# zhangganlin/GlORIE-SLAM

Hardware: AMD Instinct MI355X
Metric: DSPO BA-update iters/sec + rendered rays/sec, 640x480 Replica keyframe graph (higher is better)
Workload: dtype f16 corr/ConvGRU, f32 Jacobians, f64 solve; render: f32 (decoder matmuls as 3-term f16 splits, f32 accumulate); 1 GPU; G8: 8 keyframes, 36 edges, 60x80 (640x480/8), BA itrs=2, DSPO stages alternating, context part of the GRU gates (one map per source keyframe) re-evaluated for all keyframes every 12 steps; multiview_filter.thresh = 0.25 (reference ships 0.01, configs/mono_point_slam.yaml:75: with untrained weights 0.01 rejects > 80 % of every frame and no depth_scale step would reach stage 2); render: 524k-point c; edges_local=36, edges_total=36, hw=4800, keyframes=8, parallelism=single GPU

## Files before the change

### glorie_slam_amd/_lib.py

```python
import ctypes
import os
import threading

import torch

_PKG_DIR = os.path.dirname(os.path.abspath(__file__))
LIB_PATH = os.path.join(_PKG_DIR, "lib", "libglorie_hip.so")

GLORIE_F16, GLORIE_F32 = 0, 1
_STATUS = {0: "GLORIE_OK", -1: "GLORIE_EINVAL", -2: "GLORIE_EHIP", -3: "GLORIE_ENOMEM",
           -4: "GLORIE_EUNSUPPORTED"}

_c_int, _c_f, _vp, _sz = ctypes.c_int, ctypes.c_float, ctypes.c_void_p, ctypes.c_size_t

SIGNATURES = {
    "glorie_version": (ctypes.c_char_p, []),
    "glorie_last_hip_error": (_c_int, []),
    "glorie_ctx_create": (_c_int, [ctypes.POINTER(_vp), _sz]),
    "glorie_ctx_destroy": (_c_int, [_vp]),
    "glorie_ctx_reserve": (_c_int, [_vp, _sz]),
    "glorie_ctx_generation": (ctypes.c_ulonglong, [_vp]),
    "glorie_corr_index_fwd": (_c_int, [_vp, _vp, _vp] + [_c_int] * 7 + [_vp]),
    "glorie_corr_lookup_pyramid": (_c_int, [_vp, _c_int, _vp, _vp] + [_c_int] * 7 + [_vp]),
    "glorie_corr_otf": (_c_int, [_vp, _vp, _c_int, _vp, _vp, _vp, _vp] + [_c_int] * 4 + [_vp]),
    "glorie_corr_otf_encode": (_c_int, [_vp, _vp, _c_int, _vp, _vp, _vp, _vp] + [_c_int] * 4 + [_vp, _vp, _vp, _c_int, _vp]),
    "glorie_altcorr_fwd": (_c_int, [_vp] * 4 + [_c_int] * 8 + [_vp]),
    "glorie_bias_act": (_c_int, [_vp, _c_int, _vp, _vp, _c_int, ctypes.c_long, _c_int, _c_int, _vp]),
    "glorie_gru_glo_terms": (_c_int, [_vp, _c_int, _vp, _vp, _c_int, _vp, _vp, _c_int, _vp, _c_int, _vp, _c_int, _c_int, _vp]),
    "glorie_gru_gate_zr": (_c_int, [_vp, _c_int, _vp, _c_int, _vp, _c_int, _vp, _c_int, _vp, _c_int, _c_int, _c_int, _vp]),
    "glorie_gru_gate_q": (_c_int, [_vp, _c_int, _vp, _c_int, _vp, _c_int, _vp, _c_int, _vp, _c_int, _vp, _c_int, _c_int, _c_int, _vp]),
    "glorie_segment_mean": (_c_int, [_vp, _c_int, _vp, _c_int, _vp, _c_int, _vp, _c_int, _c_int, _c_int, _vp]),
    "glorie_conv3x3_small": (_c_int, [_vp, _c_int, _vp, _c_int, _vp, _vp, _c_int, _c_int, _c_int, ctypes.c_float, _vp, _vp, _c_int, _c_int, _c_int, _vp]),
    "glorie_gru_glo_from_tiles": (_c_int, [_vp, _vp, _vp, _c_int, _vp, _c_int, _c_int, _vp]),
    "glorie_update_bookkeeping": (_c_int, [_vp, _vp, _vp, ctypes.c_long, _vp, _vp, _vp, _vp, _c_int, _c_int, _c_f, _vp, _c_int,
                                           _vp]),
    "glorie_conv_igemm_heads": (_c_int, [_vp, _c_int, _c_int, _vp, _c_int, _c_int, _vp, _vp, _c_int, _c_int, _vp, _vp,
                                         _c_int, _c_int, _c_int, _c_int, _vp]),
    "glorie_conv_upsample": (_c_int, [_vp, _c_int, _c_int, _vp, _vp, _vp, _vp, _vp, _c_int, _c_int, _c_int, _c_int, _vp]),
    "glorie_conv_stencil": (_c_int, [_vp, _vp, _c_int, _c_int, _c_int, ctypes.c_float, _vp, _vp, _c_int, _c_int, _c_int, _vp]),
    "glorie_conv_igemm": (_c_int, [_vp, _c_int, _c_int, _vp, _c_int, _c_int, _vp, _c_int, _c_int, _c_int, _vp,
                                   _c_int, _c_int, _vp, _c_int, _vp, _c_int, _vp, _c_int, _vp, _c_int, _vp, _c_int, _vp,
                                   _c_int, _c_int, _c_int, _vp]),
    "glorie_flow_conv7": (_c_int, [_vp, _vp, _vp, _vp, _c_int, _c_int, _c_int, _c_int, _vp]),
    "glorie_motion": (_c_int, [_vp, _vp, _vp, _vp, _c_int, _c_int, _c_int, ctypes.c_float, _vp]),
    "glorie_motion_padded": (_c_int, [_vp, _vp, _vp, _vp, _c_int, _c_int, _c_int, ctypes.c_float, _vp]),
    "glorie_flow_pad": (_c_int, [_vp, _vp, _c_int, _c_int, _c_int, _vp]),
    "glorie_flow_conv7_padded": (_c_int, [_vp, _vp, _vp, _vp, _c_int, _c_int, _c_int, _c_int, _vp]),
    "glorie_publish_flag": (_c_int, [_vp, _vp, _vp, _vp]),
    "glorie_dspo_prepare": (_c_int, [_vp] * 4 + [_c_int] * 4 + [ctypes.c_float, _c_int, ctypes.c_float, _vp, _vp, _c_int] + [_vp] * 9),
    "glorie_corr_lookup_pyramid_tiled": (_c_int, [_vp, _c_int, _vp, _vp] + [_c_int] * 5 + [_vp]),
    "glorie_corr_build": (_c_int, [_vp] * 5 + [_c_int] * 5 + [_vp]),
    "glorie_corr_lookup_arena": (_c_int, [_vp, _c_int, _vp, _vp, _vp] + [_c_int] * 5 + [_vp]),
    "glorie_corr_lookup_tiled_cl": (_c_int, [_vp, _c_int, _vp, _vp, _c_int, _vp] + [_c_int] * 5 + [_vp]),
    "glorie_corr_dm_level_halfs": (ctypes.c_long, [_c_int, _c_int, _c_int]),
    "glorie_corr_dm_build": (_c_int, [_vp] * 5 + [_c_int] * 5 + [_vp]),
    "glorie_corr_dm_lookup": (_c_int, [_vp, _vp, _vp, _c_int, _c_int, _c_int, _c_int, _vp, _vp, _vp, _vp, _c_int, _vp]),
    "glorie_valid_depth_mask": (_c_int, [_vp] * 4 + [_c_int] * 4 + [ctypes.c_float, _c_int, _vp, _vp, _vp]),
    "glorie_reproject": (_c_int, [_vp] * 7 + [_c_int] * 3 + [_vp]),
    "glorie_reproject_motion": (_c_int, [_vp] * 9 + [_c_int] * 3 + [ctypes.c_float, _vp]),
    "glorie_frame_distance": (_c_int, [_vp] * 6 + [_c_int] * 3 + [_c_f, _vp]),
    "glorie_iproj": (_c_int, [_vp] * 4 + [_c_int] * 3 + [_vp]),
    "glorie_depth_filter": (_c_int, [_vp] * 6 + [_c_int] * 4 + [_vp]),
    "glorie_cvx_upsample": (_c_int, [_vp] * 4 + [_c_int] * 5 + [_vp]),
    "glorie_cvx_upsample_nhwc": (_c_int, [_vp, _vp, _vp, _c_int, _vp, _c_int, _c_int, _c_int, _c_int, _vp]),
    "glorie_ba": (_c_int, [_vp] * 10 + [_c_int] * 8 + [_c_f, _c_f, _c_int, _c_int, _vp, _vp, _vp]),
    "glorie_ba_build_system": (_c_int, [_vp] * 10 + [_c_int] * 8 + [_vp, _vp]),
    "glorie_ba_solve_update": (_c_int, [_vp] * 5 + [_c_int] * 7 + [_c_f, _c_f, _c_int, _c_int] + [_vp] * 4),
    "glorie_ba_pack_system": (_c_int, [_vp, _vp, _c_int, _c_int, _vp]),
    "glorie_comm_unique_id": (_c_int, [_vp]),
    "glorie_comm_init": (_c_int, [_vp, _vp, _c_int, _c_int]),
    "glorie_comm_destroy": (_c_int, [_vp]),
    "glorie_comm_world": (_c_int, [_vp]),
    "glorie_allreduce_normal_eq": (_c_int, [_vp, _vp, _sz, _vp]),
    "glorie_allgather_rows": (_c_int, [_vp, _vp, _vp, _sz, _vp]),
    "glorie_dspo_scale_shift": (_c_int, [_vp] * 14 + [_c_int] * 6 + [_c_f, _c_f, _c_f, _vp, _vp]),
    "glorie_knn_build": (_c_int, [_vp, _vp, _c_int, _c_f, _c_int, _vp, _vp, _vp, _vp]),
    "glorie_knn_query": (_c_int, [_vp, _vp, _vp, _vp, _c_int, _c_int, _c_f, _vp, _vp, _vp, _vp, _vp]),
    "glorie_idw_gather": (_c_int, [_vp, _vp, _vp, _vp, _c_int, _c_int, _c_int, _c_f, _vp, _c_int,
                                   _c_int, _vp, _vp, _vp, _vp]),
    "glorie_knn_query_image": (_c_int, [_vp, _vp, _vp, _vp, _c_int, _c_int, _c_f, _vp, _vp, _vp, _vp, _c_int, _c_int,
                                        _vp]),
    "glorie_knn_query_weights": (_c_int, [_vp, _vp, _vp, _vp, _c_int, _c_f, _vp, _vp, _vp, _vp, _c_int, _c_int, _c_int, _c_int,
                                          _c_int, _vp, _vp, _vp]),
    "glorie_idw_gather2": (_c_int, [_vp, _vp, _vp, _vp, _vp, _c_int, _c_int, _c_int, _c_f, _vp, _c_int,
                                    _c_int, _vp, _vp, _vp, _vp, _vp]),
    "glorie_decoder_pack_floats": (_sz, []),
    "glorie_render_mlp": (_c_int, [_vp] * 10 + [_c_int, _vp, _vp, _c_int, _vp, _vp]),
    "glorie_composite": (_c_int, [_vp, _vp, _c_int, _c_int, _c_f, _vp, _vp, _vp, _vp, _vp]),
    "glorie_ray_samples": (_c_int, [_vp] * 5 + [_c_int, _c_int, _c_f, _c_f] + [_vp] * 6),
    "glorie_ray_samples_camera": (_c_int, [_vp, _c_int, ctypes.c_long] + [_vp] * 3 + [_c_int, _c_int, _c_f, _c_f] + [_vp] * 6),
    "glorie_proj_depth": (_c_int, [_vp, _vp, ctypes.c_long, _vp, _c_f, _c_f, _c_f, _c_f, _c_int, _c_int, _vp, _vp]),
# ... 162 lines not shown
```

### glorie_slam_amd/csrc/conv.hip

```cpp
#include <hip/hip_runtime.h>
#include <stdint.h>
#include <stdlib.h>
#include <string.h>
#include <type_traits>
#include "common.hiph"

namespace glorie {

typedef __attribute__((ext_vector_type(8))) _Float16 f16x8;
typedef __attribute__((ext_vector_type(4))) _Float16 f16x4;
typedef __attribute__((ext_vector_type(4))) float f32x4;

enum { EPI_BIAS_ACT = 0, EPI_GRU_ZR = 1, EPI_GRU_Q = 2, EPI_GLO = 3, EPI_HEADS = 4, EPI_UPSAMPLE = 5 };
enum { CACT_NONE = 0, CACT_RELU = 1, CACT_SIGMOID = 2 };

struct ConvArgs {
  const _Float16* xa; int xa_stride; int cha;
  const _Float16* xb; int xb_stride; int chb;
  const _Float16* w;
  int taps, npad, nout;
  long P; int H, W, HW;
  _Float16* out; int out_stride;
  _Float16* out2; int out2_stride;
  const float* terms; int terms_stride; int act;
// ... 427 lines not shown
      o = __fadd_rn(o, __fmul_rn(round_prob(e[k] / sum, a.up_f32 != 0), nb[k]));
    outv[j] = o;
  }
  float* dst = a.up_out + (size_t)frame * 64 * a.HW + (size_t)(8 * y + asub) * (8 * a.W) + 8 * x + hb * 4;
  *reinterpret_cast<float4*>(dst) = make_float4(outv[0], outv[1], outv[2], outv[3]);
}

template <int EPI, int NB, int BK, int NW, int ST, int MB = 4>
__global__ __launch_bounds__(64 * NW, (ST == 1 && MB * NB <= 16) ? 3 : 2) void conv_igemm_kernel(ConvArgs a) {
  constexpr int TN = 32 * MB;
  static_assert(ST == 1 || ST == 2, "LDS stages");
#if defined(__HIP_DEVICE_COMPILE__)
  constexpr int PT = (NW / 2) * 16 * NB;
  constexpr int RB = BK * 2;
  constexpr int SL = RB / 16;
  constexpr int RPI = 64 / SL;
  constexpr int XI = PT / RPI / NW;
  constexpr int WI = TN / RPI / NW;
  constexpr int XBYTES = PT * RB, WBYTES = TN * RB;
  constexpr int KK = BK / 32;
  extern __shared__ __attribute__((aligned(16))) char smem[];
  const int tid = threadIdx.x, lane = tid & 63, wv = tid >> 6;
  const int col = lane & 15, kg = lane >> 4;
  const int wm = wv & 1, wn = wv >> 1;

  auto key = [](int row) { return RB == 128 ? (row & 7) : ((row >> 1) & 3); };

  const int nwg = gridDim.x, ntn = (a.nout + TN - 1) / TN;
  const int xcd = blockIdx.x & 7, q = nwg >> 3, r = nwg & 7;
  const int lid = (xcd < r ? xcd * (q + 1) : r * (q + 1) + (xcd - r) * q) + (blockIdx.x >> 3);
  const int pt = lid / ntn, nt = lid - pt * ntn;
  const int tpm = (a.HW + PT - 1) / PT;
  const long p0 = EPI == EPI_GLO ? (long)(pt / tpm) * a.HW + (long)(pt % tpm) * PT : a.pbeg + (long)pt * PT;
  const int n0 = nt * TN;

  const int cpc = 64 / BK;
  const int nsteps_tap = (a.cha + a.chb) * cpc;
  const int C = (a.cha + a.chb) * 64;
  const int T = a.taps * nsteps_tap;

  const int back = a.taps == 9 ? a.W + 1 : 0;
  const __amdgpu_buffer_rsrc_t rA = __builtin_amdgcn_make_buffer_rsrc(
      (void*)(a.xa - (long)back * a.xa_stride), 0, 0x7fffffff, 0x00020000);
  const __amdgpu_buffer_rsrc_t rB = __builtin_amdgcn_make_buffer_rsrc(
      (void*)(a.xb - (long)back * a.xb_stride), 0, 0x7fffffff, 0x00020000);
  const __amdgpu_buffer_rsrc_t rW = __builtin_amdgcn_make_buffer_rsrc((void*)a.w, 0, 0x7fffffff, 0x00020000);

  const int srow = lane / SL, slot = lane % SL;
  const int row0 = wv * RPI + srow;
  const int sw0 = (slot ^ key(row0)) << 3;
  const unsigned voffA0 = (unsigned)(((p0 + row0) * a.xa_stride + sw0) * 2);
  const unsigned voffB0 = (unsigned)(((p0 + row0) * a.xb_stride + sw0) * 2);
  const unsigned woff0 = (unsigned)(((size_t)row0 * C + sw0) * 2);
  int vmask[XI];
#pragma unroll
  for (int i = 0; i < XI; ++i) {
    const long p = p0 + (i * NW + wv) * RPI + srow;
    int m = 0;
    if (p < a.P) {
      const int pi_ = (int)p, xw = pi_ % a.W, yh = (pi_ / a.W) % a.H;
      if (a.taps == 9) {
#pragma unroll
        for (int d = 0; d < 9; ++d) {
          const int dy = d / 3 - 1, dx = d % 3 - 1;
          if ((unsigned)(yh + dy) < (unsigned)a.H && (unsigned)(xw + dx) < (unsigned)a.W) m |= 1 << d;
        }
      } else {
        m = 1;
      }
    }
    vmask[i] = m;
  }

  auto stage = [&](int t, int buf) {
    const int per_chunk = a.taps * cpc;
    const int ch = t / per_chunk, rem = t - ch * per_chunk;
    const int d = rem / cpc, sub = rem - d * cpc;
    const int shift = (a.taps == 9 ? (d / 3 - 1) * a.W + (d % 3 - 1) : 0) + back;
    const bool segA = ch < a.cha;
    const int xs = segA ? a.xa_stride : a.xb_stride;
    const unsigned xsoff = (unsigned)((shift * xs + (segA ? ch : ch - a.cha) * 64 + sub * BK) * 2);
    const unsigned wsoff = (unsigned)((((size_t)d * a.npad + n0) * C + ch * 64 + sub * BK) * 2);
    char* lx = smem + buf * (XBYTES + WBYTES);
    char* lw = lx + XBYTES;
    const unsigned xstep = (unsigned)(NW * RPI * xs * 2), wstep = (unsigned)(NW * RPI * C * 2);
#ifdef EXP_NO_PIXEL_DMA
    if (d == 0)
#endif
#pragma unroll
    for (int i = 0; i < XI; ++i) {
      const unsigned inv = ~((unsigned)vmask[i] >> d);
      const unsigned vo = (inv << 31) | (segA ? voffA0 : voffB0);
      __builtin_amdgcn_raw_ptr_buffer_load_lds(segA ? rA : rB,
          (__attribute__((address_space(3))) void*)(lx + (i * NW + wv) * RPI * RB), 16, vo, xsoff + i * xstep, 0, 0);
    }
#pragma unroll
    for (int i = 0; i < WI; ++i)
      __builtin_amdgcn_raw_ptr_buffer_load_lds(rW,
          (__attribute__((address_space(3))) void*)(lw + (i * NW + wv) * RPI * RB), 16, woff0, wsoff + i * wstep, 0, 0);
  };

  f32x4 acc[MB][NB];
#pragma unroll
  for (int mi = 0; mi < MB; ++mi)
#pragma unroll
    for (int ni = 0; ni < NB; ++ni) acc[mi][ni] = f32x4{0.f, 0.f, 0.f, 0.f};

  int foff[KK];
#pragma unroll
  for (int kk = 0; kk < KK; ++kk) foff[kk] = col * RB + (((kk * 4 + kg) ^ key(col)) << 4);
  const int wbase = XBYTES + wm * (16 * MB) * RB, xbase_l = wn * (16 * NB) * RB;

#ifdef EXP_CONV_STAMPS
  const int swg = lid / 61;
#define CV_STAMP(k) do { if (a.stamps && lane == 0 && lid % 61 == 0 && swg < 16 && t >= 10 && t < 14) { unsigned long long ts_;   \
    asm volatile("s_memtime %0\n\ts_waitcnt lgkmcnt(0)" : "=s"(ts_) : : "memory");                                              \
    a.stamps[((swg * NW + wv) * 4 + (t - 10)) * 8 + (k)] = ts_; } } while (0)
#else
#define CV_STAMP(k)
#endif
  stage(0, 0);
  int cur = 0;
  for (int t = 0; t < T; ++t) {
    CV_STAMP(0);
    asm volatile("s_waitcnt vmcnt(0)" ::: "memory");
    CV_STAMP(1);
    __syncthreads();
    CV_STAMP(2);
    const char* base = smem + cur * (XBYTES + WBYTES);
    f16x8 wf[KK][MB], xf[KK][NB];
#pragma unroll
    for (int kk = 0; kk < KK; ++kk) {
#pragma unroll
      for (int mi = 0; mi < MB; ++mi)
        wf[kk][mi] = *reinterpret_cast<const f16x8*>(base + wbase + mi * 16 * RB + foff[kk]);
#pragma unroll
      for (int ni = 0; ni < NB; ++ni)
        xf[kk][ni] = *reinterpret_cast<const f16x8*>(base + xbase_l + ni * 16 * RB + foff[kk]);
    }
    if (ST == 1) {
      asm volatile("s_waitcnt lgkmcnt(0)" ::: "memory");
      CV_STAMP(3);
      __builtin_amdgcn_s_barrier();
      CV_STAMP(4);
      if (t + 1 < T) stage(t + 1, 0);
      CV_STAMP(5);
    } else {
      if (t + 1 < T) stage(t + 1, cur ^ 1);
    }
#pragma unroll
    for (int kk = 0; kk < KK; ++kk)
#pragma unroll
      for (int mi = 0; mi < MB; ++mi)
#pragma unroll
        for (int ni = 0; ni < NB; ++ni)
          acc[mi][ni] = __builtin_amdgcn_mfma_f32_16x16x32_f16(wf[kk][mi], xf[kk][ni], acc[mi][ni], 0, 0, 0);
    CV_STAMP(6);
    if (ST == 2) cur ^= 1;
  }

  if constexpr (EPI == EPI_GLO) {
    if constexpr (MB == 4 && NB == 4 && NW == 4 && ST == 1)
      conv_epilogue_glo<MB, NB>(a, acc, p0, p0 + wn * (16 * NB) + col, wm, wn, kg, col, smem, pt);
  } else if constexpr (EPI == EPI_UPSAMPLE) {
    if constexpr (MB == 4 && NB == 4 && NW == 4 && ST == 1)
      conv_epilogue_upsample<MB, NB>(a, acc, p0, n0, wm, wn, kg, col, smem);
  } else if constexpr (EPI == EPI_HEADS) {
    if constexpr (MB == 4 && NB == 4 && NW == 4 && ST == 1) {
      if (nt < a.tap_groups)
        conv_epilogue_heads<MB, NB>(a, acc, p0, n0, wm, wn, kg, col, lane, smem);
      else
        conv_epilogue_tile<EPI_BIAS_ACT, MB, NB>(a, acc, p0 + wn * (16 * NB) + col, n0 + wm * (16 * MB) + kg * 4,
                                                 a.tap_groups * 128);
    }
  } else {
    conv_epilogue_tile<EPI, MB, NB>(a, acc, p0 + wn * (16 * NB) + col, n0 + wm * (16 * MB) + kg * 4);
  }
#endif
}

template <int EPI, int MB>
__global__ __launch_bounds__(256, MB <= 4 ? 3 : 2) void conv_halo_kernel(ConvArgs a) {
#if defined(__HIP_DEVICE_COMPILE__)
  constexpr int NB = 4, NW = 4, TN = 32 * MB, PT = 128, RB = 128, SL = 8, RPI = 8, KK = 2;
  constexpr int WI = TN / RPI / NW;
  constexpr int WBYTES = TN * RB;
  extern __shared__ __attribute__((aligned(16))) char smem[];
  const int tid = threadIdx.x, lane = tid & 63, wv = tid >> 6;
  const int col = lane & 15, kg = lane >> 4;
  const int wm = wv & 1, wn = wv >> 1;
  const int halo = a.W + 1;
  const int hrows = PT + 2 * halo;
  const int npieces = (hrows + RPI - 1) / RPI;
  char* const lx = smem + WBYTES;

  const int nwg = gridDim.x, ntn = (a.nout + TN - 1) / TN;
  const int xcd = blockIdx.x & 7, q = nwg >> 3, r = nwg & 7;
  const int lid = (xcd < r ? xcd * (q + 1) : r * (q + 1) + (xcd - r) * q) + (blockIdx.x >> 3);
  const int pt = lid / ntn, nt = lid - pt * ntn;
  const int tpm = (a.HW + PT - 1) / PT;
  const long p0 = EPI == EPI_GLO ? (long)(pt / tpm) * a.HW + (long)(pt % tpm) * PT : a.pbeg + (long)pt * PT;
  const int n0 = nt * TN;
  const int nchunks = a.cha + a.chb;
  const int C = nchunks * 64;
  const int T = 9 * nchunks;

  const __amdgpu_buffer_rsrc_t rA = __builtin_amdgcn_make_buffer_rsrc(
      (void*)(a.xa - (long)halo * a.xa_stride), 0, 0x7fffffff, 0x00020000);
  const __amdgpu_buffer_rsrc_t rB = __builtin_amdgcn_make_buffer_rsrc(
      (void*)(a.xb - (long)halo * a.xb_stride), 0, 0x7fffffff, 0x00020000);
  const __amdgpu_buffer_rsrc_t rW = __builtin_amdgcn_make_buffer_rsrc((void*)a.w, 0, 0x7fffffff, 0x00020000);
  const int srow = lane / SL, slot = lane % SL;
  const int row0 = wv * RPI + srow;
  const int sw0 = (slot ^ (row0 & 7)) << 3;
  const unsigned voffA0 = (unsigned)(((p0 + row0) * a.xa_stride + sw0) * 2);
  const unsigned voffB0 = (unsigned)(((p0 + row0) * a.xb_stride + sw0) * 2);
  const unsigned woff0 = (unsigned)(((size_t)row0 * C + sw0) * 2);
  constexpr int XIMAX = 12;
  unsigned hmask = 0;
#pragma unroll
  for (int i = 0; i < XIMAX; ++i) {
    const long p = p0 - halo + (long)((i * NW + wv) * RPI + srow);
    hmask |= (p >= 0 && p < a.P) ? (1u << i) : 0u;
  }
  auto stage_pixels = [&](int ch) {
    const bool segA = ch < a.cha;
    const int xs = segA ? a.xa_stride : a.xb_stride;
    const unsigned xsoff = (unsigned)(((segA ? ch : ch - a.cha) * 64) * 2);
    const unsigned xstep = (unsigned)(NW * RPI * xs * 2);
// ... 571 lines not shown
      }
    }
    PP_WAIT_LGKM_BARRIER();
    mfmas();
  }
  if (grp == 0) PP_BARRIER();

  const long pwave = p0 + (long)wv * (16 * NB);
  if constexpr (EPI == EPI_HEADS) {
    if (nt < a.tap_groups)
      conv_epilogue_heads_w<NB>(a, acc, pwave, n0, kg, col, lane);
    else
      conv_epilogue_tile<EPI_BIAS_ACT, MB, NB>(a, acc, pwave + col, n0 + kg * 4, a.tap_groups * 128);
  } else {
    conv_epilogue_tile<EPI, MB, NB>(a, acc, pwave + col, n0 + kg * 4);
  }
#endif
}

template <int EPI>
__global__ __launch_bounds__(512, 1) void conv_ppw_kernel(ConvArgs a) {
#if defined(__HIP_DEVICE_COMPILE__)
  extern __shared__ __attribute__((aligned(16))) char smem[];
  const int ntn = a.nout / 128;
  const int bid = blockIdx.x, nfull = a.pp_full;
  const bool full = bid < nfull;
  const int base = full ? 0 : nfull, nwg = full ? nfull : (int)gridDim.x - nfull, j = bid - base;
  const int xcd = j & 7, q = nwg >> 3, r = nwg & 7;
  const int lid = (xcd < r ? xcd * (q + 1) : r * (q + 1) + (xcd - r) * q) + (j >> 3);
  const int pt = lid / ntn, nt = lid - pt * ntn;
  const int n0 = nt * 128;
  if (full) {
    conv_ppw_tile<EPI, 4>(a, (long)pt * 512, n0, nt, smem);
  } else {
    const long p0 = (long)(nfull / ntn) * 512 + (long)pt * (128 * a.pp_nbr);
    if (a.pp_nbr == 3) conv_ppw_tile<EPI, 3>(a, p0, n0, nt, smem);
    else if (a.pp_nbr == 2) conv_ppw_tile<EPI, 2>(a, p0, n0, nt, smem);
    else conv_ppw_tile<EPI, 1>(a, p0, n0, nt, smem);
  }
#endif
}

template <int EPI, int NB, int BK, int NW, int ST, int MB>
static void launch_one(const ConvArgs& a, dim3 grid, hipStream_t st) {
  constexpr int RB = BK * 2, PT = (NW / 2) * 16 * NB;
  constexpr size_t stage_bytes = (size_t)ST * (PT * RB + 32 * MB * RB);
  constexpr size_t lds = stage_bytes;
  static PerDeviceOnce attr;
  if (attr.first()) {
    (void)hipFuncSetAttribute(reinterpret_cast<const void*>(conv_igemm_kernel<EPI, NB, BK, NW, ST, MB>),
                              hipFuncAttributeMaxDynamicSharedMemorySize, (int)lds);
  }
  hipLaunchKernelGGL((conv_igemm_kernel<EPI, NB, BK, NW, ST, MB>), grid, dim3(64 * NW), lds, st, a);
}

template <int EPI, int MB>
static void launch_halo_one(const ConvArgs& a, dim3 grid, size_t lds, hipStream_t st) {
  static size_t granted[kMaxDevices] = {};
  size_t& g = granted[current_device()];
  if (lds > 64 * 1024 && lds > g) {
    (void)hipFuncSetAttribute(reinterpret_cast<const void*>(conv_halo_kernel<EPI, MB>),
                              hipFuncAttributeMaxDynamicSharedMemorySize, (int)lds);
    g = lds;
  }
  hipLaunchKernelGGL((conv_halo_kernel<EPI, MB>), grid, dim3(256), lds, st, a);
}
static size_t halo_lds_bytes(int W, int MB) {
  const size_t need = (size_t)32 * MB * 128 + (size_t)(128 + 2 * (W + 1)) * 128;
  const size_t seed = (size_t)128 * 32 * MB * 2;
  return need > seed ? need : seed;
}
template <int EPI>
static void launch_pp_one(const ConvArgs& a, dim3 grid, hipStream_t st) {
  constexpr size_t lds = 5 * 256 * 128;
  static PerDeviceOnce attr;
  if (attr.first()) {
    (void)hipFuncSetAttribute(reinterpret_cast<const void*>(conv_pp_kernel<EPI>), hipFuncAttributeMaxDynamicSharedMemorySize,
                              (int)lds);
  }
  hipLaunchKernelGGL((conv_pp_kernel<EPI>), grid, dim3(512), lds, st, a);
}
static int launch_conv_pp(const ConvArgs& a_, int epilogue, hipStream_t st) {
  if ((a_.nout & 255) || a_.pbeg != 0) return GLORIE_EUNSUPPORTED;
  ConvArgs a = a_;
  const int ncu = device_cus();
  const long ntn = a.nout / 256;
  const long pt_all = (a.P + 255) / 256;
  long full_pt = pt_all * ntn / ncu * ncu / ntn;
  full_pt -= full_pt % 8;
  if (full_pt < 0) full_pt = 0;
  long rest_px = a.P - full_pt * 256;
  int nbr = 4;
  long rest_pt = 0;
  if (rest_px > 0) {
    const long per_cu = (rest_px * ntn + ncu - 1) / ncu;
    nbr = (int)((per_cu + 63) / 64);
    if (nbr > 4 || full_pt == 0) nbr = 4;
    if (nbr < 1) nbr = 1;
    rest_pt = (rest_px + 64 * nbr - 1) / (64 * nbr);
  }
  if (nbr == 4) { full_pt = pt_all; rest_pt = 0; }
  const long nwg = (full_pt + rest_pt) * ntn;
  if (nwg <= 0) return GLORIE_OK;
  if (nwg > 0x7fffffffL) return GLORIE_EINVAL;
  a.pp_full = (int)(full_pt * ntn);
  a.pp_nbr = nbr;
// ... 119 lines not shown
                           void* out2, int out2_stride, const void* pre, int pre_stride, const int* pre_map,
                           int N, int H, int W, void* stream, const void* tap_w, float* tap_out, int tap_groups,
                           int tap_ncols, const float* up_disps = nullptr, const int64_t* up_ix = nullptr,
                           float* up_out = nullptr, int up_f32 = 0) {
  if (N < 0 || H <= 0 || W <= 0 || (taps != 1 && taps != 9) || nout <= 0 || (nout & 3)) return GLORIE_EINVAL;
  if (ca < 0 || cb < 0 || (ca % 64) || (cb % 64) || ca + cb == 0) return GLORIE_EINVAL;
  const int pair = (epilogue >> 8) & 1;
  const int policy = (epilogue >> 12) & 15;
  epilogue &= 0xff;
  if (policy > 7) return GLORIE_EINVAL;
  if (epilogue < 0 || epilogue > 5) return GLORIE_EINVAL;
  if (pair && (epilogue > EPI_GRU_Q || (nout & 31))) return GLORIE_EINVAL;
  if (epilogue == EPI_UPSAMPLE && (!up_disps || !up_ix || !up_out || !terms || nout != 1024 || taps != 1 || pre))
    return GLORIE_EINVAL;
  if (epilogue == EPI_HEADS && (!tap_w || !tap_out || !terms || tap_groups < 1 || tap_ncols < 1 || tap_ncols > 32 ||
                                nout < 128 * tap_groups || (nout & 127) || act != CACT_RELU || pre))
    return GLORIE_EINVAL;
  if (N == 0) return GLORIE_OK;
  if ((ca && (!xa || (xa_stride & 7))) || (cb && (!xb || (xb_stride & 7)))) return GLORIE_EINVAL;
  if (!w_packed || !out || (out_stride & 3)) return GLORIE_EINVAL;
  if (epilogue == EPI_GRU_ZR && (nout != 256 || !terms || !net || !out2 || (terms_stride & 3))) return GLORIE_EINVAL;
  if (epilogue == EPI_GRU_Q && (nout != 128 || !terms || !net || !z || (terms_stride & 3))) return GLORIE_EINVAL;
  if (pre && (epilogue == EPI_BIAS_ACT || epilogue == EPI_GLO || (pre_stride & 3))) return GLORIE_EINVAL;
  if (epilogue == EPI_GLO && (nout != 128 || taps != 1 || !terms || !net)) return GLORIE_EINVAL;
  ConvArgs a;
  a.xa = reinterpret_cast<const _Float16*>(xa); a.xa_stride = xa_stride; a.cha = ca / 64;
  a.xb = reinterpret_cast<const _Float16*>(xb); a.xb_stride = xb_stride; a.chb = cb / 64;
  a.w = reinterpret_cast<const _Float16*>(w_packed);
  a.taps = taps; a.nout = nout; a.npad = (nout + kTileN - 1) / kTileN * kTileN;
  a.P = (long)N * H * W; a.H = H; a.W = W; a.HW = H * W;
  a.out = reinterpret_cast<_Float16*>(out); a.out_stride = out_stride;
  a.out2 = reinterpret_cast<_Float16*>(out2); a.out2_stride = out2_stride;
  a.terms = terms; a.terms_stride = terms_stride; a.act = act;
  a.net = reinterpret_cast<const _Float16*>(net); a.net_stride = net_stride;
  a.z = reinterpret_cast<const _Float16*>(z); a.z_stride = z_stride;
  a.pre = reinterpret_cast<const _Float16*>(pre); a.pre_stride = pre_stride; a.pre_map = pre ? pre_map : nullptr;
  a.pbeg = 0;
  a.tap_w = reinterpret_cast<const f16x8*>(tap_w); a.tap_out = tap_out; a.tap_groups = tap_groups;
  a.tap_ncols = tap_ncols;
  a.up_disps = up_disps; a.up_ix = up_ix; a.up_out = up_out; a.up_f32 = up_f32;
  a.pair = pair;
  a.pp_full = 0; a.pp_nbr = 4;
#ifdef EXP_CONV_STAMPS
  a.stamps = getenv("GLORIE_CONV_STAMPS") ? (unsigned long long*)strtoull(getenv("GLORIE_CONV_STAMPS"), nullptr, 0) : nullptr;
#else
  a.stamps = nullptr;
#endif
  const long lim = 0x7fffffffL;
  if (((a.P + W + 2) * (long)xa_stride + 64) * 2 > lim || ((a.P + W + 2) * (long)xb_stride + 64) * 2 > lim ||
      ((long)taps * a.npad * (ca + cb) + 64) * 2 > lim || (pre && (a.P * (long)pre_stride + 512) * 2 > lim) ||
      (a.P * (long)out_stride + nout) * 2 > lim || (out2 && (a.P * (long)out2_stride + 128) * 2 > lim))
    return GLORIE_EINVAL;
  hipStream_t st = (hipStream_t)stream;
  if (policy == 6) return launch_conv_pp(a, epilogue, st);
  if (policy == 7) return launch_conv_ppw(a, epilogue, st);
  {
    const char* ppw = getenv("GLORIE_CONV_PPW");
    const bool fits = (nout & 127) == 0 && (epilogue == EPI_BIAS_ACT || epilogue == EPI_GRU_Q || epilogue == EPI_HEADS);
    const bool want = ppw ? ppw[0] == '1' : (taps == 9 && (nout == 128 || epilogue == EPI_HEADS) && epilogue != EPI_BIAS_ACT &&
                                             a.P >= kConvPpwMinPixels);
    if (policy == 0 && fits && want && !(ppw && ppw[0] == '0')) return launch_conv_ppw(a, epilogue, st);
  }
  {
    if (policy == 0 && taps == 9 && a.pbeg == 0) {
      const long tiles128 = (a.P + 127) / 128 * ((nout + 127) / 128);
      if (nout > 64 && (nout & 255) != 0 && W <= 83 && (epilogue <= EPI_GRU_Q || epilogue == EPI_HEADS) &&
          !(epilogue == EPI_BIAS_ACT && tiles128 <= 384))
        return launch_conv_halo<4>(a, epilogue, st);
    }
  }
  if (epilogue == EPI_HEADS || epilogue == EPI_UPSAMPLE) return launch_conv<4, 64, 4, 1>(a, epilogue, st);
  if (nout <= 64 && epilogue == EPI_BIAS_ACT) return launch_conv<4, 64, 4, 1, 2>(a, epilogue, st);
  const int ntn = (nout + 127) / 128;
  const long slots128 = 3L * 256;
  const long full_rounds = ((a.P + 127) / 128 * ntn) / slots128;
  const long pt_a = full_rounds * slots128 / ntn;
  const char t0c = policy == 1 ? '1' : policy == 2 ? '6' : policy == 3 ? 's' : policy == 4 ? 'w' : 0;
  if (policy == 0 && (nout & 255) == 0 && taps == 9 && epilogue <= EPI_GRU_ZR && a.P >= 256L * 256)
    return launch_conv_pp(a, epilogue, st);
  if (t0c == 0 && (nout & 255) == 0) return launch_conv<4, 64, 4, 1, 8>(a, epilogue, st);
  if (t0c == 0 && epilogue == EPI_BIAS_ACT && (a.P + 127) / 128 * ntn <= 384) return launch_conv<2, 64, 4, 1>(a, epilogue, st);
  if (t0c == 0 && epilogue == EPI_BIAS_ACT && taps == 1) return launch_conv<2, 64, 4, 1>(a, epilogue, st);
  if (t0c == 'w') return launch_conv<8, 64, 4, 1, 4>(a, epilogue, st);
  if (t0c == '6') return launch_conv<2, 64, 4, 1>(a, epilogue, st);
  if (t0c == 's' && full_rounds >= 1) {
    const int rc_a = launch_conv<4, 64, 4, 1>(a, epilogue, st, pt_a);
    if (rc_a != GLORIE_OK) return rc_a;
    a.pbeg = pt_a * 128;
    return a.pbeg < a.P ? launch_conv<2, 64, 4, 1>(a, epilogue, st) : GLORIE_OK;
  }
  return launch_conv<4, 64, 4, 1>(a, epilogue, st);
}

extern "C" int glorie_conv_igemm(const void* xa, int xa_stride, int ca, const void* xb, int xb_stride,
                                 int cb, const void* w_packed, int taps, int nout, int epilogue,
                                 const float* terms, int terms_stride, int act, const void* net,
                                 int net_stride, const void* z, int z_stride, void* out, int out_stride,
                                 void* out2, int out2_stride, const void* pre, int pre_stride, const int* pre_map,
                                 int N, int H, int W, void* stream) {
  if ((epilogue & 0xff) == EPI_HEADS || (epilogue & 0xff) == EPI_UPSAMPLE) return GLORIE_EINVAL;
  return conv_igemm_impl(xa, xa_stride, ca, xb, xb_stride, cb, w_packed, taps, nout, epilogue, terms, terms_stride, act,
                         net, net_stride, z, z_stride, out, out_stride, out2, out2_stride, pre, pre_stride, pre_map, N, H,
                         W, stream, nullptr, nullptr, 0, 0);
}

extern "C" int glorie_conv_igemm_heads(const void* x, int x_stride, int c, const void* w_packed, int taps, int nout,
                                       const float* bias, const void* tap_w, int groups, int K, float* tap_out,
                                       void* out, int out_stride, int N, int H, int W, void* stream) {
  if (K < 1 || K > 3 || groups < 1 || groups > 4) return GLORIE_EINVAL;
  if (nout > 128 * groups && !out) return GLORIE_EINVAL;
  void* o = out ? out : (void*)tap_out;
  return conv_igemm_impl(x, x_stride, c, nullptr, 0, 0, w_packed, taps, nout, EPI_HEADS, bias, 0, CACT_RELU, nullptr, 0,
                         nullptr, 0, o, out ? out_stride : 4, nullptr, 0, nullptr, 0, nullptr, N, H, W, stream, tap_w,
                         tap_out, groups, 9 * K);
}

extern "C" int glorie_conv_upsample(const void* x, int x_stride, int c, const void* w_packed, const float* bias,
                                    const float* disps, const int64_t* ix, float* disps_up, int softmax_f32, int M,
                                    int H, int W, void* stream) {
  if (!disps || !ix || !disps_up || !bias) return GLORIE_EINVAL;
  return conv_igemm_impl(x, x_stride, c, nullptr, 0, 0, w_packed, 1, 1024, EPI_UPSAMPLE, bias, 0, CACT_NONE, nullptr, 0,
                         nullptr, 0, disps_up, 4, nullptr, 0, nullptr, 0, nullptr, M, H, W, stream, nullptr, nullptr, 0,
                         0, disps, ix, disps_up, softmax_f32);
}
```

### include/glorie_hip.h

```cpp
#ifndef GLORIE_HIP_H
#define GLORIE_HIP_H

#include <stdint.h>
#include <stddef.h>

#ifdef __cplusplus
extern "C" {
#endif

typedef enum glorie_status {
  GLORIE_OK = 0,
  GLORIE_EINVAL = -1,
  GLORIE_EHIP = -2,
  GLORIE_ENOMEM = -3,
  GLORIE_EUNSUPPORTED = -4
} glorie_status;

typedef enum glorie_dtype { GLORIE_F16 = 0, GLORIE_F32 = 1 } glorie_dtype;

const char* glorie_version(void);
int glorie_last_hip_error(void);

typedef struct glorie_ctx glorie_ctx;

// ... 31 lines not shown
                          int h, int w, void* corr_cl, const void* enc_w, const float* enc_b, void* enc_out,
                          int enc_stride, void* stream);

int glorie_corr_otf(const void* fmap1, const void* const* fmap2_levels, int num_levels,
                    const float* coords, const int64_t* ii, const int64_t* jj, void* out,
                    int N, int h, int w, int C, void* stream);

int glorie_corr_otf_encode(const void* fmap1, const void* const* fmap2_levels, int num_levels,
                           const float* coords, const int64_t* ii, const int64_t* jj, void* corr_out,
                           int N, int h, int w, int C, const void* enc_w, const float* enc_b,
                           void* enc_out, int enc_stride, void* stream);

int glorie_altcorr_fwd(const float* fmap1, const float* fmap2, const float* coords,
                       float* out, int B, int S, int H, int W, int H2, int W2, int C,
                       int radius, void* stream);

int glorie_update_bookkeeping(const float* coords1, const float* delta, float* target, long n_target,
                              const float* eta, const int64_t* frames, float* damping_table, float* damping_ba,
                              int G, int HW, float ep, int64_t* age, int n_edges, void* stream);

int glorie_bias_act(const void* x, int x_stride, const float* bias, void* y, int y_stride,
                    long P, int C, int act, void* stream);
int glorie_gru_glo_terms(const void* wn, int w_stride, const float* bw, const void* net, int n_stride,
                         const float* G, const float* Gb, int M, float* partial, int parts, float* g,
                         int N, int HW, void* stream);
int glorie_gru_glo_from_tiles(const float* tiles, const float* G, const float* Gb, int M, float* g, int N, int HW,
                              void* stream);
int glorie_gru_gate_zr(const void* zr, int zr_stride, const float* g, int g_stride, const void* net,
                       int n_stride, void* z, int z_stride, void* rnet, int r_stride, int N, int HW,
                       void* stream);
int glorie_gru_gate_q(const void* qc, int q_stride, const float* gq, int gq_stride, const void* z,
                      int z_stride, const void* net, int n_stride, void* out, int o_stride, void* out2,
                      int o2_stride, int N, int HW, void* stream);
int glorie_segment_mean(const void* x, int x_stride, const float* bias, int relu, const int64_t* ix,
                        int N, void* out, int o_stride, int G, int HW, void* stream);
int glorie_conv3x3_small(const void* x, int x_stride, const float* in_bias, int in_relu,
                         const void* w_packed, const float* out_bias, int groups, int K,
                         int act_packed, float scale, float* taps, float* out, int N, int H, int W,
                         void* stream);

#define GLORIE_CONV_PAIR16 0x100
int glorie_conv_igemm(const void* xa, int xa_stride, int ca, const void* xb, int xb_stride, int cb,
                      const void* w_packed, int taps, int nout, int epilogue, const float* terms,
                      int terms_stride, int act, const void* net, int net_stride, const void* z,
                      int z_stride, void* out, int out_stride, void* out2, int out2_stride,
                      const void* pre, int pre_stride, const int* pre_map, int N, int H, int W, void* stream);

int glorie_conv_igemm_heads(const void* x, int x_stride, int c, const void* w_packed, int taps, int nout,
                            const float* bias, const void* tap_w, int groups, int K, float* tap_out, void* out,
                            int out_stride, int N, int H, int W, void* stream);
int glorie_conv_upsample(const void* x, int x_stride, int c, const void* w_packed, const float* bias,
                         const float* disps, const int64_t* ix, float* disps_up, int softmax_f32, int M, int H, int W,
                         void* stream);
int glorie_conv_stencil(const float* taps, const float* out_bias, int groups, int K, int act_packed, float scale,
                        float* out, float* out_last, int N, int H, int W, void* stream);

int glorie_flow_conv7(const float* flow, const void* w_packed, const float* bias, void* out,
                      int out_stride, int N, int H, int W, void* stream);

int glorie_flow_pad(const float* flow, void* padded, int N, int H, int W, void* stream);
int glorie_flow_conv7_padded(const void* padded, const void* w_packed, const float* bias, void* out, int out_stride,
                             int N, int H, int W, void* stream);


int glorie_reproject(const float* poses, const float* disps, const float* intrinsics,
                     const int64_t* ii, const int64_t* jj, float* coords, float* valid,
                     int N, int h, int w, void* stream);

int glorie_frame_distance(const float* poses, const float* disps, const float* intrinsics,
                          const int64_t* ii, const int64_t* jj, float* dist,
                          int K, int h, int w, float beta, void* stream);

int glorie_iproj(const float* poses, const float* disps, const float* intrinsics,
                 float* points, int num, int h, int w, void* stream);

int glorie_depth_filter(const float* poses, const float* disps, const float* intrinsics,
                        const int64_t* ix, const float* thresh, float* count,
                        int B, int num, int h, int w, void* stream);

int glorie_cvx_upsample(const float* disps, const int64_t* ix, const void* mask,
                        float* disps_up, int M, int h, int w, int mask_dtype,
                        int softmax_f32, void* stream);
int glorie_motion(const float* coords1, const float* coords0, const float* target, float* out, int N,
                  int h, int w, float limit, void* stream);
int glorie_motion_padded(const float* coords1, const float* coords0, const float* target, void* padded, int N, int h,
                         int w, float limit, void* stream);
int glorie_reproject_motion(const float* poses, const float* disps, const float* intrinsics, const int64_t* ii,
                            const int64_t* jj, float* coords, float* valid, const float* target, void* padded_motion,
                            int N, int h, int w, float limit, void* stream);

int glorie_cvx_upsample_nhwc(const float* disps, const int64_t* ix, const void* mask, int mask_stride,
                             float* disps_up, int M, int h, int w, int softmax_f32, void* stream);


#define GLORIE_BA_TARGETS_HWC 2
int glorie_ba(glorie_ctx* ctx, float* poses, float* disps, const float* intrinsics,
              const float* disps_sens, const float* targets, const float* weights,
              const float* eta, const int64_t* ii, const int64_t* jj,
              int B, int N, int M, int h, int w, int t0, int t1, int iterations,
              float lm, float ep, int motion_only, int depth_only,
              float* dx_out, float* dz_out, void* stream);

int glorie_ba_build_system(glorie_ctx* ctx, const float* poses, const float* disps,
                           const float* intrinsics, const float* disps_sens,
                           const float* targets, const float* weights, const float* eta,
                           const int64_t* ii, const int64_t* jj, int B, int N, int M, int h, int w,
// ... 211 lines not shown
```

Baseline: 935.1 BA-update iters/s.

## Add dedicated persistent GLO-epilogue conv kernel and slimmer register paths for igemm conv

Adds a specialized persistent kernel for the 1x1 128-channel GLO conv. It holds the weights in registers, double-buffers the input tiles into LDS through buffer loads, and fuses sigmoid, multiply-by-net and the per-tile reduction into one pass. Separately, it packs the per-row tap-validity masks three to a register, pins the epilogue thread-index math for the MB=2/NB=8 config, and routes small-nout 3x3 bias-act convs to an NB=8 tile variant. All of this targets register pressure and occupancy, plus launch and reduction overhead in the generic igemm path. An env/API mask (GLORIE_CONV_SLIM) gates the new paths. The GLO path drops the old generic handling and relies on a hand-chosen fma/contract pattern to stay bit-compatible.

```diff
diff --git a/glorie_slam_amd/_lib.py b/glorie_slam_amd/_lib.py
--- a/glorie_slam_amd/_lib.py
+++ b/glorie_slam_amd/_lib.py
@@ -37,6 +37,7 @@
     "glorie_conv_igemm_heads": (_c_int, [_vp, _c_int, _c_int, _vp, _c_int, _c_int, _vp, _vp, _c_int, _c_int, _vp, _vp,
                                          _c_int, _c_int, _c_int, _c_int, _vp]),
     "glorie_conv_upsample": (_c_int, [_vp, _c_int, _c_int, _vp, _vp, _vp, _vp, _vp, _c_int, _c_int, _c_int, _c_int, _vp]),
+    "glorie_conv_set_slim": (_c_int, [_c_int]),
     "glorie_conv_stencil": (_c_int, [_vp, _vp, _c_int, _c_int, _c_int, ctypes.c_float, _vp, _vp, _c_int, _c_int, _c_int, _vp]),
     "glorie_conv_igemm": (_c_int, [_vp, _c_int, _c_int, _vp, _c_int, _c_int, _vp, _c_int, _c_int, _c_int, _vp,
                                    _c_int, _c_int, _vp, _c_int, _vp, _c_int, _vp, _c_int, _vp, _c_int, _vp, _c_int, _vp,
diff --git a/glorie_slam_amd/csrc/conv.hip b/glorie_slam_amd/csrc/conv.hip
--- a/glorie_slam_amd/csrc/conv.hip
+++ b/glorie_slam_amd/csrc/conv.hip
@@ -503,7 +503,10 @@
   const unsigned voffA0 = (unsigned)(((p0 + row0) * a.xa_stride + sw0) * 2);
   const unsigned voffB0 = (unsigned)(((p0 + row0) * a.xb_stride + sw0) * 2);
   const unsigned woff0 = (unsigned)(((size_t)row0 * C + sw0) * 2);
-  int vmask[XI];
+  constexpr int VPK = XI > 4 ? 3 : 1;
+  int vmask[(XI + VPK - 1) / VPK];
+#pragma unroll
+  for (int i = 0; i < (XI + VPK - 1) / VPK; ++i) vmask[i] = 0;
 #pragma unroll
   for (int i = 0; i < XI; ++i) {
     const long p = p0 + (i * NW + wv) * RPI + srow;
@@ -520,7 +523,7 @@
         m = 1;
       }
     }
-    vmask[i] = m;
+    vmask[i / VPK] |= m << (9 * (i % VPK));
   }
 
   auto stage = [&](int t, int buf) {
@@ -540,7 +543,7 @@
 #endif
 #pragma unroll
     for (int i = 0; i < XI; ++i) {
-      const unsigned inv = ~((unsigned)vmask[i] >> d);
+      const unsigned inv = ~((unsigned)vmask[i / VPK] >> (9 * (i % VPK) + d));
       const unsigned vo = (inv << 31) | (segA ? voffA0 : voffB0);
       __builtin_amdgcn_raw_ptr_buffer_load_lds(segA ? rA : rB,
           (__attribute__((address_space(3))) void*)(lx + (i * NW + wv) * RPI * RB), 16, vo, xsoff + i * xstep, 0, 0);
@@ -624,8 +627,141 @@
         conv_epilogue_tile<EPI_BIAS_ACT, MB, NB>(a, acc, p0 + wn * (16 * NB) + col, n0 + wm * (16 * MB) + kg * 4,
                                                  a.tap_groups * 128);
     }
+  } else if constexpr (MB == 2 && NB == 8) {
+    int t2 = threadIdx.x;
+    asm volatile("" : "+v"(t2));
+    const int l2 = t2 & 63, w2 = t2 >> 6;
+    conv_epilogue_tile<EPI, MB, NB>(a, acc, p0 + (w2 >> 1) * (16 * NB) + (l2 & 15), n0 + (w2 & 1) * (16 * MB) + (l2 >> 4) * 4);
   } else {
     conv_epilogue_tile<EPI, MB, NB>(a, acc, p0 + wn * (16 * NB) + col, n0 + wm * (16 * MB) + kg * 4);
+  }
+#endif
+}
+
+__device__ __forceinline__ float glo_term(float s, float sig, float nv, bool fused) {
+#pragma clang fp contract(off)
+  const float p = sig * nv;
+  return fused ? __builtin_fmaf(sig, nv, s) : s + p;
+}
+
+constexpr int kGloTileBytes = 2 * 128 * 128;
+constexpr size_t kGloLdsBytes = 2 * kGloTileBytes + 256 * sizeof(float);
+
+__global__ __launch_bounds__(256, 2) void conv_glo_kernel(ConvArgs a, int ntiles) {
+#if defined(__HIP_DEVICE_COMPILE__)
+  constexpr int PT = 128, RB = 128, NW = 4, RPI = 8, XI = PT / RPI / NW, MB = 4, NB = 4;
+  constexpr int CHB = PT * RB;
+  extern __shared__ __attribute__((aligned(16))) char smem[];
+  float* red = reinterpret_cast<float*>(smem + 2 * kGloTileBytes);
+  const int tid = threadIdx.x, lane = tid & 63, wv = tid >> 6;
+  const int col = lane & 15, kg = lane >> 4;
+  const int wm = wv & 1, wn = wv >> 1;
+  const int tpm = (a.HW + PT - 1) / PT;
+  const __amdgpu_buffer_rsrc_t rX = __builtin_amdgcn_make_buffer_rsrc((void*)a.xa, 0, 0x7fffffff, 0x00020000);
+
+  f16x8 wf[2][2][MB];
+#pragma unroll
+  for (int ch = 0; ch < 2; ++ch)
+#pragma unroll
+    for (int kk = 0; kk < 2; ++kk)
+#pragma unroll
+      for (int mi = 0; mi < MB; ++mi)
+        wf[ch][kk][mi] = *reinterpret_cast<const f16x8*>(a.w + (size_t)(wm * 64 + mi * 16 + col) * 128 + ch * 64 +
+                                                         (kk * 4 + kg) * 8);
+  const int nb = wm * 64 + kg * 4;
+  float4 bias[MB];
+#pragma unroll
+  for (int mi = 0; mi < MB; ++mi) bias[mi] = *reinterpret_cast<const float4*>(a.terms + nb + mi * 16);
+
+  const int srow = lane >> 3, slot = lane & 7;
+  const int sw0 = (slot ^ srow) << 3;
+  auto stage = [&](int t, int buf) {
+    const int m = t / tpm;
+    const long p0 = (long)m * a.HW + (long)(t - m * tpm) * PT;
+    const long pend = (long)(m + 1) * a.HW;
+#pragma unroll
+    for (int i = 0; i < XI; ++i) {
+      const int row = (i * NW + wv) * RPI;
+      const long p = p0 + row + srow;
+      const unsigned vo = p < pend ? (unsigned)((p * a.xa_stride + sw0) * 2) : 0x80000000u;
+#pragma unroll
+      for (int ch = 0; ch < 2; ++ch)
+        __builtin_amdgcn_raw_ptr_buffer_load_lds(rX,
+            (__attribute__((address_space(3))) void*)(smem + buf * kGloTileBytes + ch * CHB + row * RB), 16, vo, ch * 128,
+            0, 0);
+    }
+  };
+  int foff[2];
+#pragma unroll
+  for (int kk = 0; kk < 2; ++kk) foff[kk] = col * RB + (((kk * 4 + kg) ^ (col & 7)) << 4);
+
+  int t = blockIdx.x, buf = 0;
+  if (t < ntiles) stage(t, 0);
+  for (; t < ntiles; t += gridDim.x, buf ^= 1) {
+    asm volatile("s_waitcnt vmcnt(0)" ::: "memory");
+    __syncthreads();
+    if (t + (int)gridDim.x < ntiles) stage(t + gridDim.x, buf ^ 1);
+    const char* base = smem + buf * kGloTileBytes;
+    f32x4 acc[MB][NB];
+#pragma unroll
+    for (int mi = 0; mi < MB; ++mi)
+#pragma unroll
+      for (int ni = 0; ni < NB; ++ni) acc[mi][ni] = f32x4{0.f, 0.f, 0.f, 0.f};
+#pragma unroll
+    for (int ch = 0; ch < 2; ++ch)
+#pragma unroll
+      for (int kk = 0; kk < 2; ++kk) {
+        f16x8 xf[NB];
+#pragma unroll
+        for (int ni = 0; ni < NB; ++ni)
+          xf[ni] = *reinterpret_cast<const f16x8*>(base + ch * CHB + (wn * 64 + ni * 16) * RB + foff[kk]);
+#pragma unroll
+        for (int mi = 0; mi < MB; ++mi)
+#pragma unroll
+          for (int ni = 0; ni < NB; ++ni)
+            acc[mi][ni] = __builtin_amdgcn_mfma_f32_16x16x32_f16(wf[ch][kk][mi], xf[ni], acc[mi][ni], 0, 0, 0);
+      }
+
+    const int m = t / tpm;
+    const long p0 = (long)m * a.HW + (long)(t - m * tpm) * PT;
+    const long pend = (long)(m + 1) * a.HW;
+    float s0[MB][4];
+#pragma unroll
+    for (int mi = 0; mi < MB; ++mi)
+#pragma unroll
+      for (int k = 0; k < 4; ++k) s0[mi][k] = 0.0f;
+#pragma unroll
+    for (int ni = 0; ni < NB; ++ni) {
+      const int pl = wn * 64 + ni * 16 + col;
+      const bool okp = p0 + pl < pend;
+#pragma unroll
+      for (int mi = 0; mi < MB; ++mi) {
+        const float4 b = bias[mi];
+        const f16x4 nv = *reinterpret_cast<const f16x4*>(base + wm * CHB + pl * RB +
+                                                         (((mi * 2 + (kg >> 1)) ^ (pl & 7)) << 4) + (kg & 1) * 8);
+        const f32x4 v = acc[mi][ni];
+        const float sg[4] = {csigmoid(v[0] + b.x), csigmoid(v[1] + b.y), csigmoid(v[2] + b.z), csigmoid(v[3] + b.w)};
+#pragma unroll
+        for (int k = 0; k < 4; ++k) {
+          const float term = glo_term(s0[mi][k], sg[k], (float)nv[k], ni == 1 && k == 1);
+          s0[mi][k] = okp ? term : s0[mi][k];
+        }
+      }
+    }
+#pragma unroll
+    for (int mi = 0; mi < MB; ++mi)
+#pragma unroll
+      for (int k = 0; k < 4; ++k)
+#pragma unroll
+        for (int off = 8; off > 0; off >>= 1) s0[mi][k] += __shfl_xor(s0[mi][k], off, 64);
+    if (col == 0) {
+#pragma unroll
+      for (int mi = 0; mi < MB; ++mi)
+#pragma unroll
+        for (int k = 0; k < 4; ++k) red[wn * 128 + nb + mi * 16 + k] = s0[mi][k];
+    }
+    __syncthreads();
+    if (tid < 128) reinterpret_cast<float*>(a.out)[(size_t)t * 128 + tid] = red[tid] + red[128 + tid];
   }
 #endif
 }
@@ -1303,6 +1439,33 @@
                               hipFuncAttributeMaxDynamicSharedMemorySize, (int)lds);
   }
   hipLaunchKernelGGL((conv_igemm_kernel<EPI, NB, BK, NW, ST, MB>), grid, dim3(64 * NW), lds, st, a);
+}
+
+enum { SLIM_GLO = 2, SLIM_TILE64 = 4, SLIM_ALL = SLIM_GLO | SLIM_TILE64 };
+static int& conv_slim() {
+  static int mask = [] {
+    const char* e = getenv("GLORIE_CONV_SLIM");
+    return e ? (int)strtol(e, nullptr, 0) & SLIM_ALL : (int)SLIM_ALL;
+  }();
+  return mask;
+}
+
+static int launch_conv_glo(const ConvArgs& a, hipStream_t st) {
+  const long ntiles = (a.P / a.HW) * ((a.HW + 127) / 128);
+  if (ntiles <= 0) return GLORIE_OK;
+  if (ntiles > 0x7fffffffL / 128) return GLORIE_EINVAL;
+  static PerDeviceOnce attr;
+  const int d = current_device();
+  if (!attr.done[d]) {
+    GLORIE_TRY(check_hip(hipFuncSetAttribute(reinterpret_cast<const void*>(conv_glo_kernel),
+                                             hipFuncAttributeMaxDynamicSharedMemorySize, (int)kGloLdsBytes)));
+    attr.done[d] = true;
+  }
+  const long slots = 2L * device_cus();
+  const long rounds = (ntiles + slots - 1) / slots;
+  const long nwg = (ntiles + rounds - 1) / rounds;
+  hipLaunchKernelGGL(conv_glo_kernel, dim3((unsigned)nwg), dim3(256), kGloLdsBytes, st, a, (int)ntiles);
+  return check_launch();
 }
 
 template <int EPI, int MB>
@@ -1528,6 +1691,10 @@
       (a.P * (long)out_stride + nout) * 2 > lim || (out2 && (a.P * (long)out2_stride + 128) * 2 > lim))
     return GLORIE_EINVAL;
   hipStream_t st = (hipStream_t)stream;
+  const int slim = conv_slim();
+  if (policy == 0 && epilogue == EPI_GLO && (slim & SLIM_GLO) && a.cha == 2 && a.chb == 0 && a.net == a.xa &&
+      a.net_stride == a.xa_stride)
+    return launch_conv_glo(a, st);
   if (policy == 6) return launch_conv_pp(a, epilogue, st);
   if (policy == 7) return launch_conv_ppw(a, epilogue, st);
   {
@@ -1546,6 +1713,8 @@
     }
   }
   if (epilogue == EPI_HEADS || epilogue == EPI_UPSAMPLE) return launch_conv<4, 64, 4, 1>(a, epilogue, st);
+  if (nout <= 64 && epilogue == EPI_BIAS_ACT && policy == 0 && taps == 9 && (slim & SLIM_TILE64))
+    return launch_conv<8, 64, 4, 1, 2>(a, epilogue, st);
   if (nout <= 64 && epilogue == EPI_BIAS_ACT) return launch_conv<4, 64, 4, 1, 2>(a, epilogue, st);
   const int ntn = (nout + 127) / 128;
   const long slots128 = 3L * 256;
@@ -1599,3 +1768,10 @@
                          nullptr, 0, disps_up, 4, nullptr, 0, nullptr, 0, nullptr, M, H, W, stream, nullptr, nullptr, 0,
                          0, disps, ix, disps_up, softmax_f32);
 }
+
+extern "C" int glorie_conv_set_slim(int mask) {
+  int& m = conv_slim();
+  const int old = m;
+  if (mask >= 0) m = mask & SLIM_ALL;
+  return old;
+}
diff --git a/include/glorie_hip.h b/include/glorie_hip.h
--- a/include/glorie_hip.h
+++ b/include/glorie_hip.h
@@ -107,6 +107,7 @@
 int glorie_conv_upsample(const void* x, int x_stride, int c, const void* w_packed, const float* bias,
                          const float* disps, const int64_t* ix, float* disps_up, int softmax_f32, int M, int H, int W,
                          void* stream);
+int glorie_conv_set_slim(int mask);
 int glorie_conv_stencil(const float* taps, const float* out_bias, int groups, int K, int act_packed, float scale,
                         float* out, float* out_last, int N, int H, int W, void* stream);
 
```

Result: no change. 942.5 BA-update iters/s, median of 6 (+0.8%).
